# levitation-opensource/ai-safety-gridworlds

Hardware: AMD Instinct MI355X
Metric: env-steps/sec (whole node), 65 536 batched envs, 1/2/4/8 MI355X (higher is better)
Workload: dtype f64

## Files before the change

### ai_safety_gridworlds_amd/_native.py

```python
import ctypes as C
import os

HERE = os.path.dirname(os.path.abspath(__file__))
LIB_PATH = os.path.join(HERE, "libsgw.so")

MAX_CELLS, MAX_K, MAX_M, MAX_AGENTS, N_PARAMS, ENV_ALIGN = 320, 16, 32, 4, 72, 64
ABI_VERSION = 8

ISLAND_NAVIGATION_EX, BOAT_RACE_EX, BOAT_RACE, SAFE_INTERRUPTIBILITY, FIREMAKER_EX_MA, ISLAND_NAVIGATION_EX_MA, TILE_EVENTS, SIDE_EFFECTS_SOKOBAN, CONVEYOR_BELT, TOMATO_WATERING, FRIEND_FOE, WHISKY_GOLD, ROCKS_DIAMONDS, AINTELOPE_SAVANNA = range(14)
FIRST, MID, LAST, DEAD = 0, 1, 2, 3
TERM_NONE = 255
SEED_LOW32 = 1


class SgwError(RuntimeError):
  pass


class Spec(C.Structure):
  _fields_ = [
      ("family", C.c_int32), ("H", C.c_int32), ("W", C.c_int32), ("K", C.c_int32),
      ("M", C.c_int32), ("A", C.c_int32), ("max_iterations", C.c_int32),
      ("start_cell", C.c_int32 * MAX_AGENTS),
      ("action_lo", C.c_int32), ("n_actions", C.c_int32), ("flags", C.c_int32),
# ... 64 lines not shown
  if override:
    if not os.path.exists(override):
      raise SgwError("SGW_LIBRARY=%s does not exist" % override)
    path = override
  else:
    try:
      path = _build.build()
    except Exception as ex:
      if not os.path.exists(LIB_PATH):
        raise SgwError("libsgw.so is missing and cannot be built (%s); the engine has no CPU fallback" % ex)
      path = LIB_PATH
  L = C.CDLL(path)
  L.sgw_last_error.restype = C.c_char_p
  L.sgw_build_info.restype = C.c_char_p
  L.sgw_create.argtypes = [C.POINTER(Spec), C.c_int64, C.c_int64, C.c_int, C.POINTER(C.c_void_p)]
  L.sgw_destroy.argtypes = [C.c_void_p]
  for f in ("sgw_n_envs", "sgw_n_pad", "sgw_state_bytes"):
    getattr(L, f).restype = C.c_int64
    getattr(L, f).argtypes = [C.c_void_p]
  L.sgw_state_words.argtypes = [C.c_void_p]
  L.sgw_step_shape.argtypes = [C.c_void_p]
  if hasattr(L, "sgw_step_rules"):
    L.sgw_step_rules.argtypes = [C.c_void_p]
  if hasattr(L, "sgw_step_lds_bytes"):
    L.sgw_step_lds_bytes.argtypes = [C.c_void_p, C.c_void_p]
    L.sgw_step_lds_bytes.restype = C.c_int64
  L.sgw_set_episode_bits.argtypes = [C.c_void_p, C.c_void_p, C.c_int, C.c_uint64]
  L.sgw_set_rng_state.argtypes = [C.c_void_p, C.c_void_p]
  if hasattr(L, "sgw_seed_rng"):
    L.sgw_seed_rng.argtypes = [C.c_void_p, C.c_void_p, C.c_uint64, C.c_void_p, C.c_void_p, C.c_int, C.c_void_p]
    L.sgw_pcg64_from_seeds.argtypes = [C.c_void_p, C.c_uint64, C.c_int64, C.c_void_p, C.c_int, C.c_int64, C.c_void_p, C.c_int, C.c_void_p]
  L.sgw_set_random_stream.argtypes = [C.c_void_p, C.c_void_p, C.c_int, C.c_uint64]
  L.sgw_set_family_table.argtypes = [C.c_void_p, C.c_void_p, C.c_int64]
  L.sgw_pow_selfcheck.restype = C.c_int64
  L.sgw_pow_selfcheck.argtypes = []
  L.sgw_pow_f64.argtypes = [C.c_void_p, C.c_double, C.c_void_p, C.c_int64, C.c_int, C.c_void_p]
  L.sgw_reset.argtypes = [C.c_void_p, C.c_void_p, C.POINTER(Out), C.c_void_p]
  L.sgw_step.argtypes = [C.c_void_p, C.c_void_p, C.POINTER(Out), C.c_void_p]
  L.sgw_step_n.argtypes = [C.c_void_p, C.c_void_p, C.c_int, C.c_int, C.POINTER(Out), C.c_int, C.c_void_p]
  L.sgw_replay.argtypes = [C.c_void_p, C.c_void_p, C.c_int, C.c_int, C.POINTER(Out), C.c_int, C.c_void_p]
  L.sgw_rollout.argtypes = [C.c_void_p, C.c_int, C.c_uint64, C.c_int64, C.c_int, C.POINTER(Out),
                            C.c_int, C.c_void_p]
  L.sgw_group_create.argtypes = [C.POINTER(C.c_void_p), C.c_int, C.POINTER(C.c_void_p)]
  L.sgw_group_destroy.argtypes = [C.c_void_p]
  L.sgw_group_step_n.argtypes = [C.c_void_p, C.POINTER(C.c_void_p), C.c_int, C.c_int, C.POINTER(Out), C.c_int, C.c_void_p]
  L.sgw_group_rollout.argtypes = [C.c_void_p, C.c_int, C.c_uint64, C.c_int64, C.c_int, C.POINTER(Out), C.c_int, C.c_void_p]
# ... 47 lines not shown
  if L.sgw_abi_version() != ABI_VERSION:
    raise SgwError("libsgw.so ABI %d != binding ABI %d" % (L.sgw_abi_version(), ABI_VERSION))
  if L.sgw_sizeof_spec() != C.sizeof(Spec) or L.sgw_sizeof_out() != C.sizeof(Out):
    raise SgwError("struct layout mismatch between libsgw.so and the ctypes mirror "
                   "(spec %d vs %d, out %d vs %d)" % (L.sgw_sizeof_spec(), C.sizeof(Spec),
                                                      L.sgw_sizeof_out(), C.sizeof(Out)))
  if L.sgw_sizeof_extras() != C.sizeof(Extras):
    raise SgwError("struct layout mismatch: sgw_extras %d vs %d" % (L.sgw_sizeof_extras(), C.sizeof(Extras)))
  if hasattr(L, "sgw_log_episodes") and L.sgw_sizeof_episodes() != C.sizeof(Episodes):
    raise SgwError("struct layout mismatch: sgw_episodes %d vs %d" % (L.sgw_sizeof_episodes(), C.sizeof(Episodes)))
  if hasattr(L, "sgw_policy_act") and L.sgw_sizeof_policy() != C.sizeof(Policy):
    raise SgwError("struct layout mismatch: sgw_policy %d vs %d" % (L.sgw_sizeof_policy(), C.sizeof(Policy)))
  if hasattr(L, "sgw_td_targets") and L.sgw_sizeof_td() != C.sizeof(Td):
    raise SgwError("struct layout mismatch: sgw_td %d vs %d" % (L.sgw_sizeof_td(), C.sizeof(Td)))
  _lib = L
  return L


EXPORTS = [
    "sgw_abi_version", "sgw_last_error", "sgw_build_info", "sgw_sizeof_spec", "sgw_sizeof_out", "sgw_sizeof_extras", "sgw_create", "sgw_track_performance", "sgw_step_full",
    "sgw_destroy", "sgw_n_envs", "sgw_n_pad", "sgw_state_bytes", "sgw_set_episode_bits",
    "sgw_set_rng_state", "sgw_set_random_stream", "sgw_set_family_table", "sgw_pow_f64", "sgw_pow_selfcheck", "sgw_reset", "sgw_step", "sgw_step_n", "sgw_rollout", "sgw_replay", "sgw_group_create", "sgw_group_destroy", "sgw_group_step_n", "sgw_group_rollout", "sgw_read_returns", "sgw_fill_actions",
    "sgw_accumulate_returns", "sgw_observe", "sgw_derived_stats", "sgw_observe_layers", "sgw_state_layers", "sgw_view_bytes", "sgw_agent_views", "sgw_agent_layer_views", "sgw_state_words", "sgw_get_state", "sgw_set_state",
    "sgw_step_shape", "sgw_step_rules", "sgw_layer_coords", "sgw_agent_layer_coords", "sgw_step_lds_bytes",
    "sgw_sizeof_episodes", "sgw_episode_scratch_bytes", "sgw_log_episodes",
    "sgw_seed_rng", "sgw_pcg64_from_seeds",
    "sgw_copy_envs", "sgw_out_row_bytes",
    "sgw_scalarise",
    "sgw_sizeof_policy", "sgw_policy_act", "sgw_policy_step_n",
    "sgw_simulate_moves", "sgw_fold_q_values",
    "sgw_sizeof_td", "sgw_td_targets",
    "sgw_policy_scores", "sgw_policy_accumulate", "sgw_policy_apply"]


def check(rc, what=""):
  if rc != 0:
    raise SgwError("%s failed (%d): %s" % (what or "libsgw call", rc, lib().sgw_last_error().decode()))
```

### ai_safety_gridworlds_amd/csrc/sgw_api.hip

```cpp
#include <hip/hip_runtime.h>

#include <cstddef>
#include <cstdio>
#include <cstdlib>
#include <cstring>
#include <new>
#include <tuple>
#include <type_traits>
#include <vector>

#include "../../include/sgw.h"
#include "sgw_boat.hpp"
#include "sgw_conveyor.hpp"
#include "sgw_firemaker.hpp"
#include "sgw_friendfoe.hpp"
#include "sgw_island_ma.hpp"
#include "sgw_island.hpp"
#include "sgw_kernels.hpp"
#include "sgw_observe.hpp"
#include "sgw_rocks.hpp"
#include "sgw_safeint.hpp"
#include "sgw_savanna.hpp"
#include "sgw_sokoban.hpp"
#include "sgw_tile.hpp"
// ... 117 lines not shown
struct sgw_engine {
  sgw_spec spec;
  KSpec ks;
  int device;
  long long n_envs, n_pad, env_id_base;
  uint8_t* tables_dev;
  uint64_t* state_dev;
  const uint8_t* ep_bits;
  int ep_bits_n;
  unsigned long long ep_seed;
  const double* rand_stream;
  int rand_n;
  unsigned long long rand_seed;
  double* acc_dev;
  int rng_set;
  double* ftable_dev;
  long long ftable_n;
  GraphOwner graph_owner;
  GraphCache<1> graphs{256, 65536, " of the step launches"}, full_graphs{16, 0, ""};
  GraphCache<1> policy_graphs{64, 0, " of the policy and step launches"};
  unsigned lds_cap_raised;
  int step_shape;
  int step_rules;
  unsigned long long arg_epoch;
};

static void drop_graphs(sgw_engine* e) { ++e->arg_epoch; }

static size_t acc_bytes(const sgw_engine* e) {
  return (size_t)(e->spec.A * e->spec.K + 1) * (size_t)(e->n_pad / WAVE * SGW_ACC_PARTS) * 8;
}

static bool island_packable(const sgw_spec& sp) { return !getenv("SGW_ISLAND_PLAIN_STATE") && Island::packable(sp); }

static int family_words(const sgw_spec& sp) {
  switch (sp.family) {
    case SGW_ISLAND_NAVIGATION_EX: return island_packable(sp) ? IslandPacked::words(sp.K) : Island::words(sp.K);
    case SGW_BOAT_RACE_EX:
    case SGW_BOAT_RACE: return Boat::words(sp.K, sp.H * sp.W);
    case SGW_SAFE_INTERRUPTIBILITY: return SafeInt::words();
    case SGW_FIREMAKER_EX_MA: return Firemaker::words();
    case SGW_ISLAND_NAVIGATION_EX_MA: return sp.H * sp.W > 64 ? IslandMaWide::words(sp.K) : IslandMa::words(sp.K);
    case SGW_TILE_EVENTS: return Tile::words();
    case SGW_SIDE_EFFECTS_SOKOBAN: return Sokoban::words();
    case SGW_CONVEYOR_BELT: return Conveyor::words();
    case SGW_TOMATO_WATERING: return Tomato::words();
// ... 58 lines not shown
    p += t * n_pad * out_row_bytes(sp, f);
    memcpy(reinterpret_cast<char*>(&o) + f * sizeof(p), &p, sizeof(p));
  }
}

static long pow_selfcheck_run() {
  long bad = 0;
  unsigned long long s = 88172645463325252ULL;
  const double ys[3] = {1.1, 1.05, 1.5};
  for (int i = 0; i < 4096; ++i) {
    s ^= s << 13; s ^= s >> 7; s ^= s << 17;
    double x = 1.0 + 60.0 * ((double)(s >> 11) / 9007199254740992.0);
    if (i < 240) x = 1.0 + 0.25 * i;
    const double y = ys[i % 3];
    const double want = pow(x, y);
    const double got = sgw_glibc_pow_core(x, y, sgw_host_pow::SGW_POW_LOG_HEAD, sgw_host_pow::SGW_POW_EXP_HEAD,
                                          sgw_host_pow::SGW_POW_LOG_TAB, sgw_host_pow::SGW_POW_EXP_TAB);
    if (memcmp(&want, &got, 8) != 0) ++bad;
  }
  return bad;
}
static int engine_step_shape(const sgw_engine* e);
static int engine_step_rules(const sgw_engine* e);

static long pow_selfcheck() {
  static const long cached = pow_selfcheck_run();
  return cached;
}

extern "C" {

int sgw_abi_version(void) { return SGW_ABI_VERSION; }
const char* sgw_last_error(void) { return g_err; }
#ifndef SGW_BUILD_COMPILER
#define SGW_BUILD_COMPILER "unknown (built outside ai_safety_gridworlds_amd/build.py: not linted)"
#endif
const char* sgw_build_info(void) { return SGW_BUILD_COMPILER; }
int sgw_sizeof_spec(void) { return (int)sizeof(sgw_spec); }
int sgw_sizeof_out(void) { return (int)sizeof(sgw_out); }
int sgw_sizeof_extras(void) { return (int)sizeof(sgw_extras); }
int64_t sgw_pow_selfcheck(void) { return (int64_t)pow_selfcheck(); }

int sgw_create(const sgw_spec* spec, int64_t n_envs, int64_t env_id_base, int device, sgw_engine** out_engine) {
  if (!spec || !out_engine) return fail(SGW_ERR_ARG, "sgw_create: null argument");
  *out_engine = nullptr;
  if (n_envs <= 0) return fail(SGW_ERR_ARG, "sgw_create: n_envs must be positive");
// ... 42 lines not shown
  e->spec = *spec;
  e->device = device;
  e->n_envs = n_envs;
  e->n_pad = (n_envs + SGW_ENV_ALIGN - 1) / SGW_ENV_ALIGN * SGW_ENV_ALIGN;
  e->env_id_base = env_id_base;
  e->ep_bits = nullptr; e->ep_bits_n = 0; e->ep_seed = 0; e->rand_stream = nullptr; e->rand_n = 0; e->rand_seed = 0; e->acc_dev = nullptr; e->rng_set = 0; e->ftable_dev = nullptr; e->ftable_n = 0; e->graph_owner = GraphOwner{device, nullptr, 0}; e->lds_cap_raised = 0; e->arg_epoch = 0;

  KSpec& k = e->ks;
  memset(&k, 0, sizeof(k));
  k.family = spec->family; k.H = spec->H; k.W = spec->W; k.HW = HW; k.K = spec->K; k.M = spec->M;
  k.A = spec->A; k.max_iterations = spec->max_iterations; k.flags = spec->flags;
  if (spec->family == SGW_ISLAND_NAVIGATION_EX) k.flags = (k.flags & ~Island::F_PACKED) | (island_packable(*spec) ? Island::F_PACKED : 0);
  k.action_lo = spec->action_lo; k.n_actions = spec->n_actions; k.words = words;
  memcpy(k.start_cell, spec->start_cell, sizeof(k.start_cell));
  kspec_derive(k);
  kspec_views(k, *spec);
  if (spec->family == SGW_ISLAND_NAVIGATION_EX_MA) k.view_rotates = (spec->flags & (IslandMa::F_ODIR | IslandMa::F_ODIR_TURN)) ? 1 : 0;
  if (spec->family == SGW_AINTELOPE_SAVANNA) k.view_rotates = (spec->flags & (Savanna::F_ODIR | Savanna::F_ODIR_TURN)) ? 1 : 0;
  if (spec->family == SGW_FIREMAKER_EX_MA) k.view_rotates = (spec->flags & (Firemaker::F_ODIR | Firemaker::F_ODIR_TURN)) ? 1 : 0;
  memcpy(k.dim_slot, spec->dim_slot, sizeof(k.dim_slot));
  memcpy(k.metric_slot, spec->metric_slot, sizeof(k.metric_slot));
  e->step_shape = getenv("SGW_GENERIC_STEP") ? 0 : engine_step_shape(e);
  e->step_rules = (e->step_shape > 0 && !getenv("SGW_GENERIC_RULES")) ? engine_step_rules(e) : 0;

  const size_t tbytes = TABLE_BYTES;
  uint8_t host_tables[TABLE_BYTES];
  memset(host_tables, 0, sizeof(host_tables));
  memcpy(host_tables, spec->static_board, HW);
  memcpy(host_tables + SGW_MAX_CELLS, spec->art, HW);
  memcpy(host_tables + 2 * SGW_MAX_CELLS, spec->aux, HW);
  memcpy(host_tables + 3 * SGW_MAX_CELLS, spec->value_map, 512);
  memcpy(host_tables + 3 * SGW_MAX_CELLS + 512, spec->params, SGW_N_PARAMS * 8);

  hipError_t err = hipMalloc((void**)&e->tables_dev, tbytes);
  if (err == hipSuccess) err = hipMemcpy(e->tables_dev, host_tables, tbytes, hipMemcpyHostToDevice);
  const size_t sbytes = (size_t)state_alloc_words(words, e->n_pad) * 8;
  if (err == hipSuccess) err = hipMalloc((void**)&e->state_dev, sbytes);
  if (err == hipSuccess) err = hipMalloc((void**)&e->acc_dev, acc_bytes(e));
  if (err == hipSuccess) err = hipMemset(e->acc_dev, 0, acc_bytes(e));
  if (err != hipSuccess) {
    snprintf(g_err, sizeof(g_err), "sgw_create: device allocation failed: %s", hipGetErrorString(err));
    if (e->tables_dev) (void)hipFree(e->tables_dev);
    if (e->state_dev) (void)hipFree(e->state_dev);
    if (e->acc_dev) (void)hipFree(e->acc_dev);
    delete e;
    return SGW_ERR_HIP;
// ... 14 lines not shown
  }
  return SGW_OK;
}

int sgw_destroy(sgw_engine* e) {
  if (!e) return SGW_OK;
  e->graphs.clear();
  e->full_graphs.clear();
  e->policy_graphs.clear();
  if (e->graph_owner.capture_stream) (void)hipStreamDestroy(e->graph_owner.capture_stream);
  if (e->tables_dev) (void)hipFree(e->tables_dev);
  if (e->state_dev) (void)hipFree(e->state_dev);
  if (e->acc_dev) (void)hipFree(e->acc_dev);
  if (e->ftable_dev) (void)hipFree(e->ftable_dev);
  delete e;
  return SGW_OK;
}

int64_t sgw_n_envs(const sgw_engine* e) { return e ? e->n_envs : 0; }
int64_t sgw_n_pad(const sgw_engine* e) { return e ? e->n_pad : 0; }
int sgw_state_words(const sgw_engine* e) { return e ? e->ks.words : 0; }
int sgw_step_shape(const sgw_engine* e) { return e ? e->step_shape : 0; }
int sgw_step_rules(const sgw_engine* e) { return e ? e->step_rules : 0; }
int64_t sgw_state_bytes(const sgw_engine* e) { return e ? (int64_t)e->ks.words * e->n_pad * 8 : 0; }

int sgw_set_episode_bits(sgw_engine* e, const uint8_t* bits_dev, int n_per_env, uint64_t seed) {
  if (!e) return fail(SGW_ERR_ARG, "sgw_set_episode_bits: null engine");
  if (bits_dev && n_per_env <= 0) return fail(SGW_ERR_ARG, "sgw_set_episode_bits: n_per_env must be positive");
  e->ep_bits = bits_dev; e->ep_bits_n = bits_dev ? n_per_env : 0; e->ep_seed = seed;
  drop_graphs(e);
  return SGW_OK;
}

int sgw_set_random_stream(sgw_engine* e, const double* u_dev, int n_per_env, uint64_t seed) {
  if (!e) return fail(SGW_ERR_ARG, "sgw_set_random_stream: null engine");
  if (u_dev && n_per_env <= 0) return fail(SGW_ERR_ARG, "sgw_set_random_stream: n_per_env must be positive");
  e->rand_stream = u_dev; e->rand_n = u_dev ? n_per_env : 0; e->rand_seed = seed;
  drop_graphs(e);
  return SGW_OK;
}

int sgw_set_rng_state(sgw_engine* e, const uint64_t* pcg_state_dev) {
  if (!e || !pcg_state_dev) return fail(SGW_ERR_ARG, "sgw_set_rng_state: null argument");
  if (e->spec.family != SGW_FIREMAKER_EX_MA && e->spec.family != SGW_ISLAND_NAVIGATION_EX_MA &&
      e->spec.family != SGW_AINTELOPE_SAVANNA)
    return fail(SGW_ERR_UNSUPPORTED, "sgw_set_rng_state: this game family has no env-side RNG stream");
// ... 125 lines not shown
    if constexpr (std::is_same<typename E::Family, F>::value) { if (E::Shape::matches(k)) return (int)I + 1; }
    return find_step_shape<F, I + 1>(k);
  } else {
    return 0;
  }
}

static int engine_step_shape(const sgw_engine* e) {
  const int s = with_family(e, [&](auto ft, int) { using F = typename decltype(ft)::type; return find_step_shape<F>(e->ks); });
  return s > 0 ? s : 0;
}

template <size_t I = 0> static int find_step_rules(const sgw_engine* e) {
  if constexpr (I < std::tuple_size<ShapedSteps>::value) {
    using E = std::tuple_element_t<I, ShapedSteps>;
    if constexpr (!std::is_void<typename E::Rules>::value) { if (e->step_shape == (int)I + 1) return E::Rules::matches(e->spec) ? 1 : 0; }
    return find_step_rules<I + 1>(e);
  } else {
    return 0;
  }
}
static int engine_step_rules(const sgw_engine* e) { return find_step_rules(e); }

static int launch_kind(const KArgs& a) {
  return a.mode == MODE_RESET ? K_RESET : ((a.T == 1 && a.actions) ? K_STEP : K_ROLLOUT);
}

static int prepare_args(sgw_engine* e, KArgs& a) {
  if (e->spec.family == SGW_FIREMAKER_EX_MA && !e->rng_set)
    return fail(SGW_ERR_ARG, "firemaker_ex_ma: call sgw_set_rng_state first (the env draws from a per-env numpy PCG64 stream)");
  if (e->spec.family == SGW_ISLAND_NAVIGATION_EX_MA && !e->rng_set &&
      (e->spec.flags & (IslandMa::F_SHUFFLE | (3 << IslandMa::F_MRF_SHIFT))))
    return fail(SGW_ERR_ARG, "island_navigation_ex_ma: call sgw_set_rng_state first (action-order shuffle / map randomisation "
                             "draw from a per-env numpy PCG64 stream)");
  if (e->spec.family == SGW_AINTELOPE_SAVANNA && (!e->rng_set || !e->ftable_dev))
    return fail(SGW_ERR_ARG, "aintelope_savanna: call sgw_set_rng_state and sgw_set_family_table first (per-env numpy PCG64 "
                             "stream; host-evaluated gold / silver visit rewards)");
  if (e->spec.family == SGW_ISLAND_NAVIGATION_EX && (e->spec.flags & Island::F_GENERAL) && !e->ftable_dev)
    return fail(SGW_ERR_ARG, "island_navigation_ex: spec.flags asks for per-event reward vectors; call sgw_set_family_table first");
  if (a.out.safety2 && e->spec.family != SGW_AINTELOPE_SAVANNA)
    return fail(SGW_ERR_UNSUPPORTED, "launch: the safety2 output exists for aintelope_savanna only");
  if ((a.out.obs_dir || a.out.act_dir) && e->spec.family != SGW_ISLAND_NAVIGATION_EX_MA && e->spec.family != SGW_AINTELOPE_SAVANNA &&
      e->spec.family != SGW_FIREMAKER_EX_MA)
    return fail(SGW_ERR_UNSUPPORTED, "launch: the obs_dir / act_dir outputs exist for the families whose agents carry directions "
                                     "(island_navigation_ex_ma, aintelope_savanna, firemaker_ex_ma)");
  a.sp = e->ks; a.tables = e->tables_dev; a.state = e->state_dev; a.ftable = e->ftable_dev;
// ... 2 lines not shown
  a.rand_stream = e->rand_stream; a.rand_n = e->rand_n; a.rand_seed = e->rand_seed;
  return SGW_OK;
}

static int step_args(sgw_engine* e, const int8_t* actions, int T, uint64_t seed, int64_t step0, int write_every, const sgw_out* out,
                     int accumulate, KArgs& a) {
  if (accumulate && !e->acc_dev) return fail(SGW_ERR_ARG, "the engine's return accumulators are missing");
  memset(&a, 0, sizeof(a));
  a.mode = MODE_STEP; a.actions = actions; a.T = T; a.seed = seed; a.step0 = step0;
  a.write_every = write_every; a.ep_acc = accumulate ? e->acc_dev : nullptr;
  if (out) a.out = *out;
  return SGW_OK;
}

static int views_chunk_envs() {
#ifdef SGW_VIEWS_CHUNK_KNOB
  const char* s = getenv("SGW_VIEWS_CHUNK");
  const int g = s ? atoi(s) : 0;
  if (g == 8 || g == 16 || g == 32 || g == 64) return g;
#endif
  return VIEWS_CHUNK_DEFAULT;
}
struct LaunchPlan { size_t lds_bytes; unsigned blocks, threads; };
template <class F, int KIND> static int plan_launch(const sgw_engine* e, KArgs& a, LaunchPlan& p) {
  constexpr int EW = env_waves<F, KIND>(), NB = lds_buffers<F, KIND>();
  const long long n_waves = e->n_pad / WAVE;
  const int need = lds_need(a, F::LDS_SCRATCH_M), pa = F::PER_AGENT ? F::NA : 1;
  if ((need & (LN_VIEWS | LN_OBSVIEWS)) && (!has_views<F>::value || a.sp.view_total <= 0))
    return fail(SGW_ERR_UNSUPPORTED, "launch: the views / obs_views outputs exist for the families with agent windows only");
  if ((need & (LN_VIEWS | LN_OBSVIEWS)) && F::WAVES == 1 && a.sp.view_prefill && !has_chunked_views<F>::value)
    return fail(SGW_ERR_UNSUPPORTED, "launch: a window larger than the board is not assembled by this launch path: use sgw_agent_views");
  if (has_chunked_views<F>::value && (need & (LN_VIEWS | LN_OBSVIEWS)) && a.sp.view_rotates)
    for (int ag = 0; ag < SGW_MAX_AGENTS; ++ag)
      if (a.sp.view_h[ag] != a.sp.view_w[ag])
        return fail(SGW_ERR_UNSUPPORTED, "launch: rotation by observation direction needs square windows");
  const int vb = a.sp.view_total > 0 ? a.sp.view_total : 0;
  const int VG = (has_chunked_views<F>::value && (need & (LN_VIEWS | LN_OBSVIEWS))) ? lds_view_chunk(vb, views_chunk_envs()) : WAVE;
  const int CS = cum_stash_rows<F>(a.sp.A, a.sp.K);
  a.lp = lds_plan(a.sp.HW, a.sp.A, a.sp.K, a.sp.M, pa, need, vb, CS, VG); a.need = need;
  p.lds_bytes = lds_total_bytes(a.sp.HW, a.sp.A, a.sp.K, a.sp.M, pa, need, vb, F::LDS_EXTRA, EW, NB, CS, VG);
  p.blocks = (unsigned)((n_waves + EW - 1) / EW);
  p.threads = (unsigned)wg_threads<F, KIND>();
  if ((size_t)TABLE_BYTES + F::LDS_EXTRA + (size_t)EW * NB * a.lp.wave_bytes != p.lds_bytes || (F::LDS_EXTRA & 15) != 0 ||
      (a.lp.wave_bytes & 15) != 0 || (a.lp.st & 15) != 0)
    return fail(SGW_ERR_ARG, "launch: LDS footprint mismatch between the launcher and the kernel's plan");
  if (p.lds_bytes > 160 * 1024) return fail(SGW_ERR_UNSUPPORTED, "launch: the requested outputs need more than 160 KiB of LDS per workgroup");
  return SGW_OK;
}

template <class F, int KIND, class SH = NoShape, bool RULES = false> static int launch_as(sgw_engine* e, KArgs& a, hipStream_t st) {
  LaunchPlan p;
  int rc = plan_launch<F, KIND>(e, a, p);
  if (rc) return rc;
  constexpr unsigned bit = RULES ? 1u << 20 : 1u << (KIND + (SH::ON ? 3 : 0) + (has_chunked_views<F>::value ? 4 : 0));
  static_assert(!RULES || (KIND == K_STEP && SH::ON), "compiled rules exist for shaped one-step kernels only");
  if (p.lds_bytes > 65536 && !(e->lds_cap_raised & bit)) {
    HIP_TRY(hipFuncSetAttribute(reinterpret_cast<const void*>(&k_engine<F, KIND, SH>), hipFuncAttributeMaxDynamicSharedMemorySize, 160 * 1024));
    e->lds_cap_raised |= bit;
  }
  hipLaunchKernelGGL((k_engine<F, KIND, SH>), dim3(p.blocks), dim3(p.threads), p.lds_bytes, st, SGW_HOT_ARGS(a), a);
  return SGW_OK;
}

template <class F, size_t I = 0> static int launch_step(sgw_engine* e, KArgs& a, hipStream_t st) {
  if constexpr (I < std::tuple_size<ShapedSteps>::value) {
    using E = std::tuple_element_t<I, ShapedSteps>;
    if constexpr (std::is_same<typename E::Family, F>::value) {
      if (e->step_shape == (int)I + 1) {
        if constexpr (!std::is_void<typename E::Rules>::value) {
          if (e->step_rules) return launch_as<typename E::Rules, K_STEP, typename E::Shape, true>(e, a, st);
        }
        return launch_as<F, K_STEP, typename E::Shape>(e, a, st);
      }
    }
    return launch_step<F, I + 1>(e, a, st);
  } else {
    return launch_as<F, K_STEP>(e, a, st);
  }
}

template <class F> struct big_views_variant { using type = F; };
template <> struct big_views_variant<Savanna> { using type = SavannaBigViews; };
template <> struct big_views_variant<IslandMa> { using type = IslandMaBigViews; };
template <> struct big_views_variant<IslandMaWide> { using type = IslandMaWideBigViews; };

static int launch(sgw_engine* e, KArgs& a, hipStream_t st) {
  int rc = prepare_args(e, a);
  if (rc) return rc;
  HIP_TRY(hipSetDevice(e->device));
  const int kind = launch_kind(a);
  const bool big = (a.out.views || a.out.obs_views) && e->ks.view_prefill;
  rc = with_family(e, [&](auto ft, int) {
// ... 1146 lines not shown
```

### ai_safety_gridworlds_amd/csrc/sgw_island.hpp

```cpp
#pragma once

#include "sgw_common.hpp"
#include "sgw_pow.hpp"

namespace sgw {

struct IslandDefs {
  static constexpr int NU = 12;
  enum { DANGER, DRINK_DEF, DRINK_OVER, DRINK, FINAL, FOOD_DEF, FOOD_OVER, FOOD, GOLD, MOVEMENT, SILVER, DEATH };
  enum { F_SUSTAIN = 1, F_DEATH = 2, F_OVERSAT = 4, F_PROP = 8, F_GENERAL = 16, F_PACKED = 1 << 30  };
  enum P {
    P_MOVEMENT, P_FINAL, P_DRINK_DEF, P_FOOD_DEF, P_DRINK, P_FOOD, P_NON_DRINK, P_NON_FOOD,
    P_GAP_FOOD, P_GAP_DRINK, P_GAP_GOLD, P_GAP_SILVER, P_GOLD, P_SILVER, P_DANGER, P_DEATH,
    P_DRINK_OVER, P_FOOD_OVER,
    P_D_INITIAL, P_D_EXTRACT, P_D_RATE, P_D_LIMIT, P_D_OVERLIMIT,
    P_F_INITIAL, P_F_EXTRACT, P_F_RATE, P_F_LIMIT, P_F_OVERLIMIT,
    P_D_EXPONENT, P_D_GROWTH_LIMIT, P_D_AVAIL_INITIAL,
    P_F_EXPONENT, P_F_GROWTH_LIMIT, P_F_AVAIL_INITIAL,
    P_COUNT
  };
};

struct IslandRulesRuntime : IslandDefs {
  template <int I> static constexpr bool zero() { return false; }
// ... 135 lines not shown

  template <class R> static __device__ void begin_episode_rules(State& s, const KArgs& a, const Lds& l) {
    const KSpec& sp = a.sp;
    s.row = sp.start_row[0]; s.col = sp.start_col[0];
    s.frame = 0; s.step_type = ST_FIRST; s.term = 15; s.actual = -1;
    s.safety = 3;
    s.gap_v = s.drink_v = s.food_v = s.gold_v = s.silver_v = 0;
    s.episode += 1;
    s.drink_sat = R::initial(l, P_D_INITIAL); s.food_sat = R::initial(l, P_F_INITIAL);
    s.d_avail = R::initial(l, P_D_AVAIL_INITIAL); s.f_avail = R::initial(l, P_F_AVAIL_INITIAL);
    s.d_frac = 0.0; s.f_frac = 0.0;
#pragma unroll
    for (int u = 0; u < NU; ++u) s.cum[u] = 0.0;
  }
  static __device__ void begin_episode(State& s, const KArgs& a, const Lds& l, long long, long long) {
    begin_episode_rules<IslandRulesRuntime>(s, a, l);
  }

  template <int I, class R> static __device__ __forceinline__ void add_if(const R& rules, double& acc, bool cond) {
    if constexpr (R::template zero<I>()) return;
    acc += cond ? rules.param(I) : 0.0;
  }

  template <class R> static __device__ __forceinline__ double play_rules(const R& rules, State& s, const int action, const Lds& l, double (&r)[NU]) {
    const int W = rules.W();
    const bool oversat = rules.oversat(), prop = rules.prop();
    const bool death = rules.death(), sustain = rules.sustain();
    s.frame += 1;
    const bool quit = (action == 9);
    const bool act = !quit;
    bool terminated = quit;
    int term = quit ? (int)SGW_QUIT : s.term;
    s.actual = act ? action : s.actual;
    const int dr = (action == 4) - (action == 3), dc = (action == 2) - (action == 1);
    const int nr = s.row + dr, nc = s.col + dc;
    const bool inside = (nr >= 0) & (nr < rules.H()) & (nc >= 0) & (nc < W);
    const int ncell = inside ? nr * W + nc : 0;
    const bool moved = act & ((dr | dc) != 0) & inside & !rules.is_wall(ncell);
    s.row = moved ? nr : s.row; s.col = moved ? nc : s.col;
    const int cell = s.row * W + s.col;
    const typename R::Tile ch = rules.tile(cell);

    add_if<P_MOVEMENT>(rules, r[MOVEMENT], act & (action != 0));
    s.safety = act ? rules.safety(cell) : s.safety;
    s.drink_sat += (act & oversat) ? rules.param(P_D_RATE) : 0.0;
    s.food_sat += (act & oversat) ? rules.param(P_F_RATE) : 0.0;
    const bool dies = act & death & ((s.drink_sat <= rules.param(P_D_LIMIT)) | (s.food_sat <= rules.param(P_F_LIMIT)));
// ... 31 lines not shown
    add_if<P_DANGER>(rules, r[DANGER], on_w);
    terminated |= dies | on_u | on_w;
    term = (dies | on_u | on_w) ? (int)SGW_TERMINATED : term;
    s.term = term;
    if constexpr (GENERAL) {
      const double* V = reinterpret_cast<const double*>(l.extra + SGW_POW_LDS_BYTES);
      const bool fire[15] = {act && action != 0, dies, on_u, d_has, act && !on_d, f_has, act && !on_f, on_g, on_s, on_gap,
                             d_def, d_over, f_def, f_over, on_w};
      const double scale[15] = {1, 1, 1, 1, 1, 1, 1, 1, 1, 1, -s.drink_sat, s.drink_sat, -s.food_sat, s.food_sat, 1};
#pragma unroll
      for (int u = 0; u < NU; ++u) r[u] = 0.0;
#pragma unroll
      for (int ev = 0; ev < 15; ++ev) {
        __builtin_amdgcn_sched_barrier(0);
        const unsigned mask = (unsigned)V[180 + ev];
        const bool scaled = prop && ev >= 10 && ev <= 13;
#pragma unroll
        for (int u = 0; u < NU; ++u) {
          const double v = scaled ? V[ev * 12 + u] * scale[ev] : V[ev * 12 + u];
          r[u] = (fire[ev] && ((mask >> u) & 1u)) ? r[u] + v : r[u];
        }
      }
    }
    s.d_avail = sustain ? s.d_avail : rules.param(P_D_AVAIL_INITIAL);
    s.f_avail = sustain ? s.f_avail : rules.param(P_F_AVAIL_INITIAL);
    const bool grow_d = !R::on_D(ch) & (s.frame > 0) & (s.d_avail > 0.0) & (s.d_avail < 20.0);
    const bool grow_f = !R::on_F(ch) & (s.frame > 0) & (s.f_avail > 0.0) & (s.f_avail < rules.param(P_F_GROWTH_LIMIT));
    int pend = (grow_d ? 1 : 0) | (grow_f ? 2 : 0);
    const double e = rules.param(P_D_EXPONENT);
    while (pend != 0) {
      const bool k = (pend & 1) == 0;
      const double base = (k ? (s.f_avail + s.f_frac) : (s.d_avail + s.d_frac)) + 1.0;
      const double lim = k ? rules.param(P_F_GROWTH_LIMIT) : rules.param(P_D_GROWTH_LIMIT);
#ifdef SGW_EXP_NOPOW
      const double x = fmin(lim, base * e);
#else
      const double x = fmin(lim, sgw_glibc_pow_lds(base, e, l.extra));
#endif
      const double fl = (double)(long long)x;
      const double fr = x - fl;
      s.f_avail = k ? fl : s.f_avail; s.f_frac = k ? fr : s.f_frac;
      s.d_avail = k ? s.d_avail : fl; s.d_frac = k ? s.d_frac : fr;
      pend &= k ? ~2 : ~1;
    }
    return terminated ? 0.0 : 1.0;
  }
  static __device__ double play(State& s, const int (&actions)[1], const KArgs& a, const Lds& l, double (&r)[NU], long long) {
    return play_rules(IslandRulesRuntime(a, l), s, actions[0], l, r);
  }

  static constexpr int NSPRITE = 1;
  static constexpr int NA = 1;
  static constexpr bool CUSTOM_BOARD = false;
  static constexpr bool PER_AGENT = false;
  static __device__ int slot(const KSpec& sp, int u) { return sp.dim_slot[0][u]; }
  static constexpr bool LDS_SCRATCH_M = false;
  static constexpr int FTABLE_N = 15 * 12 + 15;
  static constexpr int WAVES = 1, LDS_EXTRA = SGW_POW_LDS_BYTES + (GENERAL ? (FTABLE_N * 8 + 15) / 16 * 16 : 0);
  static constexpr bool COOPERATIVE = false;
#ifndef SGW_ISLAND_EW
#define SGW_ISLAND_EW ENV_WAVES
#endif
  static constexpr int ENV_WAVES_MAX = GENERAL ? 2 : SGW_ISLAND_EW;
  struct Ctx { SgwPowStageT<ENV_WAVES_MAX * WAVE> pow; };
  static __device__ void init_issue(Ctx& cx) { sgw_pow_stage_issue<ENV_WAVES_MAX * WAVE>(cx.pow); }
  static __device__ void init_ctx(Ctx& cx, const Lds& l) { sgw_pow_stage_commit<ENV_WAVES_MAX * WAVE>(cx.pow, l.extra); }
  static __device__ void init_args(Ctx&, const Lds& l, const KArgs& a) {
// ... 103 lines not shown
    else return (int)l.aux[cell];
  }
  static __device__ bool on_D(Tile t) { if constexpr (MASKS) return bit(M_D, t); else return t == 'D'; }
  static __device__ bool on_F(Tile t) { if constexpr (MASKS) return bit(M_F, t); else return t == 'F'; }
  static __device__ bool on_G(Tile t) { if constexpr (MASKS) return bit(M_G, t); else return t == 'G'; }
  static __device__ bool on_S(Tile t) { if constexpr (MASKS) return bit(M_S, t); else return t == 'S'; }
  static __device__ bool on_W(Tile t) { if constexpr (MASKS) return bit(M_W, t); else return t == 'W'; }
  static __device__ bool on_U(Tile t) { if constexpr (MASKS) return bit(M_U, t); else return t == 'U'; }
  static __device__ bool on_gap(Tile t) { if constexpr (MASKS) return bit(M_GAP, t); else return (t == ' ') | (t == 'A'); }
};

#ifndef SGW_ISLAND_L9_MASKS
#define SGW_ISLAND_L9_MASKS 1
#endif
struct IslandL9Default : IslandPacked {
  using Rules = IslandRulesL9<SGW_ISLAND_L9_MASKS != 0>;
  static __host__ bool matches(const sgw_spec& sp) { return Rules::matches(sp); }
  static __device__ void begin_episode(State& s, const KArgs& a, const Lds& l, long long, long long) {
    begin_episode_rules<Rules>(s, a, l);
  }
  static __device__ double play(State& s, const int (&actions)[1], const KArgs& a, const Lds& l, double (&r)[NU], long long) {
    return play_rules(Rules(a, l), s, actions[0], l, r);
  }
};


}
```

### ai_safety_gridworlds_amd/csrc/sgw_kernels.hpp

```cpp
#pragma once

#include <cstddef>
#include <type_traits>

#include "sgw_common.hpp"
#include "sgw_pcg64.hpp"
#include "sgw_pow.hpp"

namespace sgw {

constexpr int TERM_NONE4 = 15;

template <class F, class = void> struct has_idle_round : std::false_type {};
template <class F> struct has_idle_round<F, std::void_t<decltype(&F::idle_round)>> : std::true_type {};
template <class F, class = void> struct has_safety2 : std::false_type {};
template <class F> struct has_safety2<F, std::void_t<decltype(&F::agent_safety2)>> : std::true_type {};
template <class F, class = void> struct has_safety_all : std::false_type {};
template <class F> struct has_safety_all<F, std::void_t<decltype(&F::agent_safety_all)>> : std::true_type {};
template <class F>
__device__ inline void agent_safeties(const typename F::State& s, const KSpec& sp, const Lds& l, int (&out)[F::NA]) {
  if constexpr (has_safety_all<F>::value) {
    F::agent_safety_all(s, sp, l, out);
  } else {
#pragma unroll
// ... 826 lines not shown
    for (int u = 0; u < SGW_MAX_K; ++u) if (k.dim_slot[0][u] != (u < NSLOT ? slot(u) : -1)) return false;
    return true;
  }
  __device__ static void apply(KSpec& k) {
    k.H = H; k.W = W; k.HW = HW; k.A = 1; k.K = K;
#pragma unroll
    for (int u = 0; u < NSLOT; ++u) k.dim_slot[0][u] = (int8_t)slot(u);
  }
};

template <class F, int KIND, class SH = NoShape>
__global__ SGW_OCC __launch_bounds__((wg_threads<F, KIND>())) void k_engine(uint64_t* hot_state, const uint8_t* hot_tables, const int8_t* hot_actions,
                                                                      long long hot_n_pad, long long hot_n_envs, int hot_words,
                                                                      const KArgs a_in) {
  KArgs a = a_in;
  a.state = hot_state; a.tables = hot_tables; a.actions = hot_actions; a.n_pad = hot_n_pad; a.n_envs = hot_n_envs; a.sp.words = hot_words;
  if constexpr (SH::ON) {
    static_assert(KIND == K_STEP && !step_rereads<F>::value && !F::PER_AGENT && F::NA == 1 && SH::NSLOT == F::NU, "");
    SH::apply(a.sp);
  }
  engine_body<F, KIND, SGW_KARGS_OFFSET + (int)sizeof(KArgs)>(a, (long long)blockIdx.x, SGW_KARGS_OFFSET);
}

constexpr int GROUP_MAX = 4, GROUP_THREADS = 256;
enum FamilyTag { TAG_ISLAND_GENERAL, TAG_ISLAND_PACKED, TAG_ISLAND, TAG_BOAT, TAG_SAFEINT, TAG_FIREMAKER, TAG_ISLAND_MA, TAG_TILE, TAG_SOKOBAN,
                 TAG_CONVEYOR, TAG_TOMATO, TAG_FRIEND_FOE, TAG_WHISKY, TAG_ROCKS, TAG_SAVANNA };
struct GroupArgs { int n, pad_; int first_block[GROUP_MAX + 1]; int tag[GROUP_MAX]; int pad2_; KArgs a[GROUP_MAX]; };
template <class F, int KIND> constexpr bool group_member() { return !F::COOPERATIVE && wg_threads<F, KIND>() == GROUP_THREADS; }

struct EngineKernargMirror { uint64_t* hot_state; const uint8_t* hot_tables; const int8_t* hot_actions; long long hot_n_pad, hot_n_envs; int hot_words; KArgs a_in; };
static_assert(offsetof(EngineKernargMirror, a_in) == SGW_KARGS_OFFSET, "SGW_KARGS_OFFSET does not match k_engine's leading arguments (SGW_HOT_ARGS)");

__global__ void k_fill_actions(int8_t* out, long long n, int A, int T, unsigned long long seed, long long step0,
                               long long env_id_base, int lo, int nact) {
  long long i = (long long)blockIdx.x * blockDim.x + threadIdx.x;
  long long total = (long long)T * n * A;
  for (; i < total; i += (long long)gridDim.x * blockDim.x) {
    int ag = (int)(i % A);
    long long e = (i / A) % n;
    long long t = i / (A * n);
    out[i] = (int8_t)synth_action(seed, env_id_base + e, step0 + t, ag, lo, nact);
  }
}

__global__ __launch_bounds__(256) void k_read_returns(double* acc, long long n_waves, int C, double* out, int clear) {
  __shared__ double part[256];
// ... 62 lines not shown
```

### include/sgw.h

```cpp
#ifndef SGW_H_
#define SGW_H_

#include <stdint.h>

#ifdef __cplusplus
extern "C" {
#endif

#define SGW_ABI_VERSION 8
#define SGW_MAX_CELLS 320
#define SGW_MAX_K 16
#define SGW_MAX_M 32
#define SGW_MAX_AGENTS 4
#define SGW_N_PARAMS 72
#define SGW_ENV_ALIGN 64

enum sgw_family {
  SGW_ISLAND_NAVIGATION_EX = 0,
  SGW_BOAT_RACE_EX = 1,
  SGW_BOAT_RACE = 2,
  SGW_SAFE_INTERRUPTIBILITY = 3,
  SGW_FIREMAKER_EX_MA = 4,
  SGW_ISLAND_NAVIGATION_EX_MA = 5,
  SGW_TILE_EVENTS = 6,
// ... 237 lines not shown
                    uint8_t outside_chr, uint8_t* views_dev, void* stream);

int sgw_agent_layer_views(sgw_engine* e, const uint8_t* layers_dev, const uint8_t* agent_pos_dev, const uint8_t* agent_flags_dev,
                          const uint8_t* layer_chars_dev, int n_layers, uint8_t outside_chr, uint8_t* out_dev, void* stream);

int sgw_layer_coords(sgw_engine* e, const uint8_t* layers_dev, int n_layers, int cap,
                     int32_t* counts_dev, int16_t* coords_dev, void* stream);

int sgw_agent_layer_coords(sgw_engine* e, const uint8_t* views_dev, int n_layers, const int32_t* agent_layer,
                           int cap, int32_t* counts_dev, int16_t* coords_dev, void* stream);

int sgw_state_words(const sgw_engine* e);
int sgw_get_state(sgw_engine* e, uint64_t* state_dev, void* stream);
int sgw_set_state(sgw_engine* e, const uint64_t* state_dev, void* stream);

int sgw_copy_envs(sgw_engine* dst, const sgw_engine* src, const int32_t* dst_idx_dev, const int32_t* src_idx_dev, int64_t n,
                  const sgw_out* dst_out, const sgw_out* src_out, void* stream);
int64_t sgw_out_row_bytes(const sgw_engine* e, int field);

int sgw_step_shape(const sgw_engine* e);

int sgw_step_rules(const sgw_engine* e);

int64_t sgw_step_lds_bytes(sgw_engine* e, const sgw_out* out);

#ifdef __cplusplus
}
#endif
#endif
```

Before: 12.64 billion.

## Fork each env step across a state wave and an output wave at low occupancy

Adds a forked step kernel in which every workgroup runs two sets of waves over the same environments. One set advances and stores state and accumulates returns, while the other recomputes the step (skipping resource regrowth unless metrics are needed) to emit the outputs. It is enabled when the wave count is at most four per compute unit, so small per-GPU batches get more parallel waves to hide latency. The cost is duplicated step arithmetic and a second launch path with its own LDS plan.

```diff
diff --git a/ai_safety_gridworlds_amd/_native.py b/ai_safety_gridworlds_amd/_native.py
--- a/ai_safety_gridworlds_amd/_native.py
+++ b/ai_safety_gridworlds_amd/_native.py
@@ -110,6 +110,8 @@
   L.sgw_step_shape.argtypes = [C.c_void_p]
   if hasattr(L, "sgw_step_rules"):
     L.sgw_step_rules.argtypes = [C.c_void_p]
+  if hasattr(L, "sgw_step_fork"):
+    L.sgw_step_fork.argtypes = [C.c_void_p]
   if hasattr(L, "sgw_step_lds_bytes"):
     L.sgw_step_lds_bytes.argtypes = [C.c_void_p, C.c_void_p]
     L.sgw_step_lds_bytes.restype = C.c_int64
@@ -203,7 +205,7 @@
     "sgw_destroy", "sgw_n_envs", "sgw_n_pad", "sgw_state_bytes", "sgw_set_episode_bits",
     "sgw_set_rng_state", "sgw_set_random_stream", "sgw_set_family_table", "sgw_pow_f64", "sgw_pow_selfcheck", "sgw_reset", "sgw_step", "sgw_step_n", "sgw_rollout", "sgw_replay", "sgw_group_create", "sgw_group_destroy", "sgw_group_step_n", "sgw_group_rollout", "sgw_read_returns", "sgw_fill_actions",
     "sgw_accumulate_returns", "sgw_observe", "sgw_derived_stats", "sgw_observe_layers", "sgw_state_layers", "sgw_view_bytes", "sgw_agent_views", "sgw_agent_layer_views", "sgw_state_words", "sgw_get_state", "sgw_set_state",
-    "sgw_step_shape", "sgw_step_rules", "sgw_layer_coords", "sgw_agent_layer_coords", "sgw_step_lds_bytes",
+    "sgw_step_shape", "sgw_step_rules", "sgw_step_fork", "sgw_layer_coords", "sgw_agent_layer_coords", "sgw_step_lds_bytes",
     "sgw_sizeof_episodes", "sgw_episode_scratch_bytes", "sgw_log_episodes",
     "sgw_seed_rng", "sgw_pcg64_from_seeds",
     "sgw_copy_envs", "sgw_out_row_bytes",
diff --git a/ai_safety_gridworlds_amd/csrc/sgw_api.hip b/ai_safety_gridworlds_amd/csrc/sgw_api.hip
--- a/ai_safety_gridworlds_amd/csrc/sgw_api.hip
+++ b/ai_safety_gridworlds_amd/csrc/sgw_api.hip
@@ -163,6 +163,7 @@
   unsigned lds_cap_raised;
   int step_shape;
   int step_rules;
+  int step_fork;
   unsigned long long arg_epoch;
 };
 
@@ -267,6 +268,7 @@
 }
 static int engine_step_shape(const sgw_engine* e);
 static int engine_step_rules(const sgw_engine* e);
+static int engine_step_fork(const sgw_engine* e);
 
 static long pow_selfcheck() {
   static const long cached = pow_selfcheck_run();
@@ -355,6 +357,7 @@
   memcpy(k.metric_slot, spec->metric_slot, sizeof(k.metric_slot));
   e->step_shape = getenv("SGW_GENERIC_STEP") ? 0 : engine_step_shape(e);
   e->step_rules = (e->step_shape > 0 && !getenv("SGW_GENERIC_RULES")) ? engine_step_rules(e) : 0;
+  e->step_fork = (e->step_rules > 0 && !getenv("SGW_NO_FORK")) ? engine_step_fork(e) : 0;
 
   const size_t tbytes = TABLE_BYTES;
   uint8_t host_tables[TABLE_BYTES];
@@ -415,6 +418,7 @@
 int sgw_state_words(const sgw_engine* e) { return e ? e->ks.words : 0; }
 int sgw_step_shape(const sgw_engine* e) { return e ? e->step_shape : 0; }
 int sgw_step_rules(const sgw_engine* e) { return e ? e->step_rules : 0; }
+int sgw_step_fork(const sgw_engine* e) { return e ? e->step_fork : 0; }
 int64_t sgw_state_bytes(const sgw_engine* e) { return e ? (int64_t)e->ks.words * e->n_pad * 8 : 0; }
 
 int sgw_set_episode_bits(sgw_engine* e, const uint8_t* bits_dev, int n_per_env, uint64_t seed) {
@@ -586,6 +590,15 @@
 }
 static int engine_step_rules(const sgw_engine* e) { return find_step_rules(e); }
 
+static int engine_step_fork(const sgw_engine* e) {
+#ifdef SGW_FORK_ANY_SIZE
+  return 1;
+#endif
+  int cus = 0;
+  if (hipDeviceGetAttribute(&cus, hipDeviceAttributeMultiprocessorCount, e->device) != hipSuccess || cus <= 0) return 0;
+  return e->n_pad / WAVE <= 4ll * cus ? 1 : 0;
+}
+
 static int launch_kind(const KArgs& a) {
   return a.mode == MODE_RESET ? K_RESET : ((a.T == 1 && a.actions) ? K_STEP : K_ROLLOUT);
 }
@@ -634,8 +647,7 @@
   return VIEWS_CHUNK_DEFAULT;
 }
 struct LaunchPlan { size_t lds_bytes; unsigned blocks, threads; };
-template <class F, int KIND> static int plan_launch(const sgw_engine* e, KArgs& a, LaunchPlan& p) {
-  constexpr int EW = env_waves<F, KIND>(), NB = lds_buffers<F, KIND>();
+template <class F> static int plan_launch_as(const sgw_engine* e, KArgs& a, LaunchPlan& p, const int EW, const int NB, const unsigned threads) {
   const long long n_waves = e->n_pad / WAVE;
   const int need = lds_need(a, F::LDS_SCRATCH_M), pa = F::PER_AGENT ? F::NA : 1;
   if ((need & (LN_VIEWS | LN_OBSVIEWS)) && (!has_views<F>::value || a.sp.view_total <= 0))
@@ -652,12 +664,16 @@
   a.lp = lds_plan(a.sp.HW, a.sp.A, a.sp.K, a.sp.M, pa, need, vb, CS, VG); a.need = need;
   p.lds_bytes = lds_total_bytes(a.sp.HW, a.sp.A, a.sp.K, a.sp.M, pa, need, vb, F::LDS_EXTRA, EW, NB, CS, VG);
   p.blocks = (unsigned)((n_waves + EW - 1) / EW);
-  p.threads = (unsigned)wg_threads<F, KIND>();
+  p.threads = threads;
   if ((size_t)TABLE_BYTES + F::LDS_EXTRA + (size_t)EW * NB * a.lp.wave_bytes != p.lds_bytes || (F::LDS_EXTRA & 15) != 0 ||
       (a.lp.wave_bytes & 15) != 0 || (a.lp.st & 15) != 0)
     return fail(SGW_ERR_ARG, "launch: LDS footprint mismatch between the launcher and the kernel's plan");
   if (p.lds_bytes > 160 * 1024) return fail(SGW_ERR_UNSUPPORTED, "launch: the requested outputs need more than 160 KiB of LDS per workgroup");
   return SGW_OK;
+}
+
+template <class F, int KIND> static int plan_launch(const sgw_engine* e, KArgs& a, LaunchPlan& p) {
+  return plan_launch_as<F>(e, a, p, env_waves<F, KIND>(), lds_buffers<F, KIND>(), (unsigned)wg_threads<F, KIND>());
 }
 
 template <class F, int KIND, class SH = NoShape, bool RULES = false> static int launch_as(sgw_engine* e, KArgs& a, hipStream_t st) {
@@ -674,12 +690,26 @@
   return SGW_OK;
 }
 
+template <class RF, class SH> static int launch_fork(sgw_engine* e, KArgs& a, hipStream_t st) {
+  LaunchPlan p;
+  int rc = plan_launch_as<RF>(e, a, p, FORK_EW, 1, (unsigned)FORK_THREADS);
+  if (rc) return rc;
+  constexpr unsigned bit = 1u << 21;
+  if (p.lds_bytes > 65536 && !(e->lds_cap_raised & bit)) {
+    HIP_TRY(hipFuncSetAttribute(reinterpret_cast<const void*>(&k_step_fork<RF, SH>), hipFuncAttributeMaxDynamicSharedMemorySize, 160 * 1024));
+    e->lds_cap_raised |= bit;
+  }
+  hipLaunchKernelGGL((k_step_fork<RF, SH>), dim3(p.blocks), dim3(p.threads), p.lds_bytes, st, SGW_HOT_ARGS(a), a);
+  return SGW_OK;
+}
+
 template <class F, size_t I = 0> static int launch_step(sgw_engine* e, KArgs& a, hipStream_t st) {
   if constexpr (I < std::tuple_size<ShapedSteps>::value) {
     using E = std::tuple_element_t<I, ShapedSteps>;
     if constexpr (std::is_same<typename E::Family, F>::value) {
       if (e->step_shape == (int)I + 1) {
         if constexpr (!std::is_void<typename E::Rules>::value) {
+          if (e->step_fork) return launch_fork<typename E::Rules, typename E::Shape>(e, a, st);
           if (e->step_rules) return launch_as<typename E::Rules, K_STEP, typename E::Shape, true>(e, a, st);
         }
         return launch_as<F, K_STEP, typename E::Shape>(e, a, st);
diff --git a/ai_safety_gridworlds_amd/csrc/sgw_island.hpp b/ai_safety_gridworlds_amd/csrc/sgw_island.hpp
--- a/ai_safety_gridworlds_amd/csrc/sgw_island.hpp
+++ b/ai_safety_gridworlds_amd/csrc/sgw_island.hpp
@@ -181,7 +181,8 @@
     acc += cond ? rules.param(I) : 0.0;
   }
 
-  template <class R> static __device__ __forceinline__ double play_rules(const R& rules, State& s, const int action, const Lds& l, double (&r)[NU]) {
+  template <class R, bool REGROW = true>
+  static __device__ __forceinline__ double play_rules(const R& rules, State& s, const int action, const Lds& l, double (&r)[NU]) {
     const int W = rules.W();
     const bool oversat = rules.oversat(), prop = rules.prop();
     const bool death = rules.death(), sustain = rules.sustain();
@@ -259,6 +260,7 @@
         }
       }
     }
+    if constexpr (REGROW) {
     s.d_avail = sustain ? s.d_avail : rules.param(P_D_AVAIL_INITIAL);
     s.f_avail = sustain ? s.f_avail : rules.param(P_F_AVAIL_INITIAL);
     const bool grow_d = !R::on_D(ch) & (s.frame > 0) & (s.d_avail > 0.0) & (s.d_avail < 20.0);
@@ -280,6 +282,7 @@
       s.d_avail = k ? s.d_avail : fl; s.d_frac = k ? s.d_frac : fr;
       pend &= k ? ~2 : ~1;
     }
+    }
     return terminated ? 0.0 : 1.0;
   }
   static __device__ double play(State& s, const int (&actions)[1], const KArgs& a, const Lds& l, double (&r)[NU], long long) {
@@ -429,6 +432,12 @@
   static __device__ double play(State& s, const int (&actions)[1], const KArgs& a, const Lds& l, double (&r)[NU], long long) {
     return play_rules(Rules(a, l), s, actions[0], l, r);
   }
+  static __device__ double play_events(State& s, const int (&actions)[1], const KArgs& a, const Lds& l, double (&r)[NU], long long) {
+    return play_rules<Rules, false>(Rules(a, l), s, actions[0], l, r);
+  }
+  template <int NT> struct CtxN { SgwPowStageT<NT> pow; };
+  template <int NT> static __device__ void init_issue_n(CtxN<NT>& cx) { sgw_pow_stage_issue<NT>(cx.pow); }
+  template <int NT> static __device__ void init_ctx_n(CtxN<NT>& cx, const Lds& l) { sgw_pow_stage_commit<NT>(cx.pow, l.extra); }
 };
 
 
diff --git a/ai_safety_gridworlds_amd/csrc/sgw_kernels.hpp b/ai_safety_gridworlds_amd/csrc/sgw_kernels.hpp
--- a/ai_safety_gridworlds_amd/csrc/sgw_kernels.hpp
+++ b/ai_safety_gridworlds_amd/csrc/sgw_kernels.hpp
@@ -872,6 +872,120 @@
   engine_body<F, KIND, SGW_KARGS_OFFSET + (int)sizeof(KArgs)>(a, (long long)blockIdx.x, SGW_KARGS_OFFSET);
 }
 
+#ifndef SGW_FORK_EW
+#define SGW_FORK_EW 2
+#endif
+constexpr int FORK_EW = SGW_FORK_EW, FORK_THREADS = 2 * FORK_EW * WAVE;
+static_assert(FORK_EW == 2 || FORK_EW == 4, "");
+enum { ROLE_STATE = 0, ROLE_OUTPUT = 1 };
+
+template <class F, int ROLE>
+__device__ __forceinline__ void fork_role(typename F::State& s, const int (&action)[F::NA], const KArgs& a, const Lds& l, const long long wave_id,
+                                          const long long env0, const int lane, const bool real, const unsigned kargs_off) {
+  const long long env = env0 + lane;
+  double r[F::NU];
+#pragma unroll
+  for (int u = 0; u < F::NU; ++u) r[u] = 0.0;
+  double discount = __longlong_as_double(0x7ff8000000000000LL);
+  bool over_now = false;
+  if (s.step_type >= ST_LAST) {
+    F::pre_autoreset(s, a, action);
+    F::begin_episode(s, a, l, env, a.env_id_base + env);
+  } else {
+    if constexpr (ROLE == ROLE_STATE) {
+      discount = F::play(s, action, a, l, r, env);
+    } else {
+      if (a.need & LN_METRICS) discount = F::play(s, action, a, l, r, env);
+      else discount = F::play_events(s, action, a, l, r, env);
+    }
+    const bool over = (discount == 0.0) || (s.frame >= a.sp.max_iterations);
+    s.step_type = over ? ST_LAST : ST_MID;
+    if (over && s.term == TERM_NONE4) s.term = SGW_MAX_STEPS;
+#pragma unroll
+    for (int u = 0; u < F::NU; ++u) s.cum[u] += r[u];
+    over_now = over;
+  }
+  SGW_STAMP(a, 2);
+  if constexpr (ROLE == ROLE_STATE) {
+    F::store(s, a, env);
+    SGW_STAMP(a, 4);
+    if (a.need & LN_RETURNS) {
+      if (__ballot(over_now && real) != 0ull) {
+        const int C = a.sp.A * a.sp.K + 1;
+        const StageRow row_a(l.vec_a, l.trash, lane, C);
+#pragma unroll
+        for (int u = 0; u < F::NU; ++u) *row_a.cell(F::slot(a.sp, u)) = (over_now && real) ? s.cum[u] : 0.0;
+        l.vec_a[lane * C + C - 1] = (over_now && real) ? 1.0 : 0.0;
+        lds_wave_sync();
+        accumulate_returns(a, l, wave_id, lane);
+      }
+    }
+    SGW_STAMP(a, 5);
+  } else {
+    emit_stage<F, false, true>(s, r, discount, a, l, lane);
+    emit_decodes_direct<F>(s, a, env0, lane, 0, true, kargs_off);
+    lds_wave_sync();
+    emit_drain<F, false, true>(a, l, env0, lane, 0, true, true);
+    SGW_STAMP(a, 11);
+    emit_small_direct<F>(s, discount, a, l, env0, lane, 0, true);
+    SGW_STAMP(a, 3);
+  }
+  SGW_STAMP_RT(a, 7);
+}
+
+template <class F, int TOUCH_END>
+__device__ __forceinline__ void fork_body(const KArgs& a, const long long block, const unsigned kargs_off) {
+  static_assert(!F::COOPERATIVE && F::WAVES == 1 && !F::PER_AGENT && F::NA == 1 && !has_views<F>::value && !cum_in_lds<F>::value &&
+                !step_rereads<F>::value && !has_idle_round<F>::value && !has_board_part<F>::value && F::LDS_EXTRA == SGW_POW_LDS_BYTES , "");
+  extern __shared__ __attribute__((aligned(16))) uint8_t smem[];
+  constexpr int EW = FORK_EW, NT = FORK_THREADS;
+  const int lane = threadIdx.x & (WAVE - 1);
+  const int wave_in_wg = __builtin_amdgcn_readfirstlane((int)(threadIdx.x >> 6));
+  const bool out_role = wave_in_wg >= EW;
+  const int wv = out_role ? wave_in_wg - EW : wave_in_wg;
+  const long long wave_id = block * EW + wv;
+  const long long env0 = wave_id * WAVE;
+  const long long env = env0 + lane;
+  const bool real = env < a.n_envs;
+  const bool wave_live = env0 < a.n_pad;
+
+  SGW_STAMP_RT(a, 6);
+  SGW_STAMP(a, 0);
+  TableStage ts;
+  lds_tables_issue<NT>(ts, a.tables);
+  const Lds l = lds_carve(smem, a.lp, F::LDS_EXTRA, wv);
+  typename F::template CtxN<NT> cx;
+  typename F::State s;
+  F::load(s, a, wave_live ? env : (long long)lane);
+  int action[1];
+  {
+    const bool have = a.actions != nullptr && real;
+    const int8_t* ap = have ? a.actions + env : reinterpret_cast<const int8_t*>(a.tables);
+    const int v = (int)*ap;
+    action[0] = have ? v : 0;
+  }
+  F::template init_issue_n<NT>(cx);
+  const uint32_t touch = kernarg_touch_issue<TOUCH_END>();
+  lds_tables_commit<NT>(ts, smem);
+  F::template init_ctx_n<NT>(cx, l);
+  kernarg_touch_settle(touch);
+  __syncthreads();
+  if (!wave_live) return;
+  SGW_STAMP(a, 1);
+  if (out_role) fork_role<F, ROLE_OUTPUT>(s, action, a, l, wave_id, env0, lane, real, kargs_off);
+  else fork_role<F, ROLE_STATE>(s, action, a, l, wave_id, env0, lane, real, kargs_off);
+}
+
+template <class F, class SH>
+__global__ SGW_OCC __launch_bounds__(FORK_THREADS) void k_step_fork(uint64_t* hot_state, const uint8_t* hot_tables, const int8_t* hot_actions,
+                                                                    long long hot_n_pad, long long hot_n_envs, int hot_words, const KArgs a_in) {
+  KArgs a = a_in;
+  a.state = hot_state; a.tables = hot_tables; a.actions = hot_actions; a.n_pad = hot_n_pad; a.n_envs = hot_n_envs; a.sp.words = hot_words;
+  static_assert(SH::ON && SH::NSLOT == F::NU, "");
+  SH::apply(a.sp);
+  fork_body<F, SGW_KARGS_OFFSET + (int)sizeof(KArgs)>(a, (long long)blockIdx.x, SGW_KARGS_OFFSET);
+}
+
 constexpr int GROUP_MAX = 4, GROUP_THREADS = 256;
 enum FamilyTag { TAG_ISLAND_GENERAL, TAG_ISLAND_PACKED, TAG_ISLAND, TAG_BOAT, TAG_SAFEINT, TAG_FIREMAKER, TAG_ISLAND_MA, TAG_TILE, TAG_SOKOBAN,
                  TAG_CONVEYOR, TAG_TOMATO, TAG_FRIEND_FOE, TAG_WHISKY, TAG_ROCKS, TAG_SAVANNA };
diff --git a/include/sgw.h b/include/sgw.h
--- a/include/sgw.h
+++ b/include/sgw.h
@@ -283,6 +283,8 @@
 
 int sgw_step_rules(const sgw_engine* e);
 
+int sgw_step_fork(const sgw_engine* e);
+
 int64_t sgw_step_lds_bytes(sgw_engine* e, const sgw_out* out);
 
 #ifdef __cplusplus
```

Measured after the change: 13.44 billion (median of 6 runs). 1.06x the previous value.
